# peakcrosser7/spmv-samples

Hardware: NVIDIA B200
Metric: SpMV GFLOP/s and achieved HBM GB/s vs roofline at 1/2/4/8 B200 (higher is better)
Workload: dtype f32

## Files before the change

### include/spmv_b200.h

```cpp
#ifndef SPMV_B200_H_
#define SPMV_B200_H_

#include <stddef.h>
#include <stdint.h>

#ifdef __cplusplus
extern "C" {
#endif

#define SPMVB200_API __attribute__((visibility("default")))

typedef void *spmvb200_stream_t;

enum {
    SPMVB200_OK = 0,
    SPMVB200_ERR_INVALID = 1,
    SPMVB200_ERR_ALIGNMENT = 2,
    SPMVB200_ERR_CUDA = 3,
    SPMVB200_ERR_UNSUPPORTED = 4,
    SPMVB200_ERR_CUSPARSE = 5
};

enum {
    SPMVB200_KIND_MERGE = 0,
// ... 98 lines not shown
    int64_t n_rows;
    int64_t nnz;
    int64_t max_row_len;
    int64_t empty_rows;
    double mean_row_len;
    double std_row_len;
    int32_t chosen_kind;
    int32_t chosen_width;
} spmvb200_row_stats_t;
SPMVB200_API int spmvb200_row_stats(int offset_bits, int64_t n_rows, int64_t nnz, const void *Ap,
                                    spmvb200_row_stats_t *out, spmvb200_stream_t stream);

SPMVB200_API int spmvb200_set_option(const char *name, int64_t value);
SPMVB200_API int64_t spmvb200_get_option(const char *name);
SPMVB200_API int64_t spmvb200_launch_count(void);
SPMVB200_API void spmvb200_release_cache(void);

SPMVB200_API int spmvb200_gather_yardstick(int64_t x_elements, int64_t gathers, int reps,
                                           spmvb200_stream_t stream, double *best_ms);

SPMVB200_API int spmvb200_hot_x_info(const int32_t *Aj, int64_t *hot_columns, double *hot_share,
                                     double *build_ms);
SPMVB200_API int spmvb200_hot_x_table_info(const int32_t *Aj, int64_t *table_columns, double *table_share);

typedef struct spmvb200_matrix spmvb200_matrix_t;
SPMVB200_API int spmvb200_matrix_create(int offset_bits, int value_bits, int64_t n_rows,
                                        int64_t n_cols, int64_t nnz, const void *Ap_host,
                                        const int32_t *Aj_host, const void *Ax_host,
                                        spmvb200_matrix_t **out);
SPMVB200_API int spmvb200_matrix_create_from_device(int offset_bits, int value_bits, int64_t n_rows,
                                                    int64_t n_cols, int64_t nnz, const void *Ap_dev,
                                                    const int32_t *Aj_dev, const void *Ax_dev,
                                                    spmvb200_matrix_t **out);
SPMVB200_API int spmvb200_matrix_spmv_host(spmvb200_matrix_t *m, int kind, const void *x_host,
                                           void *y_host);
#define SPMVB200_MAX_SLOTS 4
SPMVB200_API int spmvb200_matrix_submit_host(spmvb200_matrix_t *m, int kind, int slot,
                                             const void *x_host, void *y_host);
SPMVB200_API int spmvb200_matrix_wait(spmvb200_matrix_t *m, int slot);
SPMVB200_API void spmvb200_matrix_destroy(spmvb200_matrix_t *m);

SPMVB200_API int spmvb200_gen_uniform_pm1(int value_bits, uint64_t seed, uint32_t stream_id,
                                          uint64_t first, int64_t count, void *out,
                                          spmvb200_stream_t stream);
SPMVB200_API int spmvb200_gen_lap2d(int offset_bits, int value_bits, int32_t grid_n, void *Ap,
                                    int32_t *Aj, void *Ax, spmvb200_stream_t stream);
// ... 56 lines not shown
```

### spmv_samples_b200/_lib.py

```python
from __future__ import annotations

import ctypes as C
import os
import subprocess

_PKG = os.path.dirname(os.path.abspath(__file__))
LIB_PATH = os.environ.get("SPMVB200_LIB") or os.path.join(_PKG, "libspmvb200.so")
CSRC = os.path.join(_PKG, "csrc")

OK = 0
KIND_MERGE, KIND_VECTOR, KIND_LIGHT, KIND_AUTO, KIND_CUSPARSE, KIND_STREAM = 0, 1, 2, 3, 4, 5
FLAG_STATIC_PATTERN = 1
SEMIRINGS = {"plus_times": 0, "min_plus": 1, "max_plus": 2, "or_and": 3}
MAX_PEERS = 8
IPC_HANDLE_BYTES = 64


class SpmvB200Error(RuntimeError):
    def __init__(self, status: int, where: str, detail: str = ""):
        self.status = status
        super().__init__(f"{where}: status {status} ({detail})")


class Args(C.Structure):
# ... 99 lines not shown
    L.spmvb200_power_run.argtypes = [C.c_void_p, C.c_int, C.POINTER(C.c_double)]
    L.spmvb200_power_sync.argtypes = [C.c_void_p]
    L.spmvb200_power_get.argtypes = [C.c_void_p, C.c_void_p, C.POINTER(C.c_double), C.POINTER(C.c_int64)]
    L.spmvb200_power_destroy.argtypes = [C.c_void_p]
    L.spmvb200_power_exchange.argtypes = [C.c_void_p]
    L.spmvb200_power_destroy.restype = None
    L.spmvb200_norm_exchange.argtypes = [C.c_int, C.c_int64, C.c_void_p, C.c_int, C.c_int, C.c_uint64,
                                         C.c_void_p, C.POINTER(C.c_void_p), C.c_void_p, C.c_void_p,
                                         C.c_void_p, C.c_void_p, C.c_void_p]
    L.spmvb200_main_kernel_time.argtypes = [C.POINTER(C.c_double), C.POINTER(C.c_int64)]
    L.spmvb200_device_malloc.argtypes = [C.c_size_t, C.POINTER(C.c_void_p)]
    L.spmvb200_device_free.argtypes = [C.c_void_p]
    L.spmvb200_matrix_spmv_host.argtypes = [C.c_void_p, C.c_int, C.c_void_p, C.c_void_p]
    L.spmvb200_matrix_submit_host.argtypes = [C.c_void_p, C.c_int, C.c_int, C.c_void_p, C.c_void_p]
    L.spmvb200_matrix_wait.argtypes = [C.c_void_p, C.c_int]
    L.spmvb200_matrix_destroy.argtypes = [C.c_void_p]
    L.spmvb200_matrix_destroy.restype = None
    L.spmvb200_ipc_export.argtypes = [C.c_void_p, C.c_char_p]
    L.spmvb200_ipc_open.argtypes = [C.c_char_p, C.POINTER(C.c_void_p)]
    L.spmvb200_ipc_close.argtypes = [C.c_void_p]
    L.spmvb200_release_cache.restype = None
    L.spmvb200_gather_yardstick.argtypes = [C.c_int64, C.c_int64, C.c_int, C.c_void_p, C.POINTER(C.c_double)]
    L.spmvb200_hot_x_table_info.argtypes = [C.c_void_p, C.POINTER(C.c_int64), C.POINTER(C.c_double)]
    L.spmvb200_hot_x_info.argtypes = [C.c_void_p, C.POINTER(C.c_int64), C.POINTER(C.c_double),
                                      C.POINTER(C.c_double)]
    for kind in ("merge", "vector", "light", "stream", "auto", "cusparse"):
        for otag, otype in (("o32", C.c_int32), ("o64", C.c_int64)):
            for vtag in ("f32", "f64"):
                fn = getattr(L, f"spmvb200_{kind}_i32_{otag}_{vtag}")
                fn.argtypes = [C.c_int32, C.c_int32, otype, C.c_void_p, C.c_void_p, C.c_void_p,
                               C.c_void_p, C.c_void_p, C.c_void_p]
                fn.restype = C.c_int
    _lib = L
    return L


def check(status: int, where: str) -> None:
    if status != OK:
        L = lib()
        detail = L.spmvb200_status_string(status).decode()
        if status in (3, 5):
            detail += ": " + L.spmvb200_last_cuda_error().decode()
        raise SpmvB200Error(status, where, detail)


def exported_symbols():
# ... 13 lines not shown
```

### spmv_samples_b200/csrc/api.cu

```cuda
#include <cstring>
#include <new>
#include <vector>

#include "common.cuh"

namespace spmvb200 {
int64_t merge_tile_items(int offset_bits);
void stats_cache_clear();
void cusparse_plan_clear();
template <typename ValT>
int gen_uniform_pm1(uint64_t, uint32_t, uint64_t, int64_t, ValT *, cudaStream_t);
template <typename OffT, typename ValT>
int gen_lap2d(int32_t, OffT *, int32_t *, ValT *, cudaStream_t);
template <typename OffT, typename ValT>
int gen_uniform_rows(int32_t, int32_t, int32_t, uint64_t, OffT *, int32_t *, ValT *, cudaStream_t);
int gen_rmat_edges(int32_t, uint64_t, uint64_t, int64_t, int32_t *, int32_t *, cudaStream_t);
template <typename OffT, typename ValT>
int coo_to_csr(int32_t, int64_t, int32_t *, int32_t *, const ValT *, OffT *, int32_t *, ValT *,
               cudaStream_t);

namespace {

inline bool aligned16(const void *p) { return (reinterpret_cast<uintptr_t>(p) & 15u) == 0; }

// ... 263 lines not shown
                              double *best_ms) {
    return gather_yardstick(x_elements, gathers, reps, static_cast<cudaStream_t>(stream), best_ms);
}

int spmvb200_hot_x_info(const int32_t *Aj, int64_t *hot_columns, double *hot_share, double *build_ms) {
    if (hot_columns) *hot_columns = 0;
    if (hot_share) *hot_share = 0.0;
    if (build_ms) *build_ms = 0.0;
    const HotPlan *plan = hot_plan_peek(Aj);
    if (plan) {
        if (hot_columns) *hot_columns = plan->K;
        if (hot_share) *hot_share = plan->hot_share;
        if (build_ms) *build_ms = plan->build_ms;
    }
    return SPMVB200_OK;
}

int spmvb200_hot_x_table_info(const int32_t *Aj, int64_t *table_columns, double *table_share) {
    if (table_columns) *table_columns = 0;
    if (table_share) *table_share = 0.0;
    if (const HotPlan *plan = hot_plan_peek(Aj)) {
        if (table_columns) *table_columns = plan->K_table;
        if (table_share) *table_share = plan->table_share;
    }
    return SPMVB200_OK;
}

}

struct spmvb200_matrix {
    int offset_bits, value_bits;
    int64_t n_rows, n_cols, nnz;
    void *Ap = nullptr, *Ax = nullptr;
    int32_t *Aj = nullptr;
    bool owns_csr = true;
    void *x[SPMVB200_MAX_SLOTS] = {}, *y[SPMVB200_MAX_SLOTS] = {};
    cudaStream_t stream[SPMVB200_MAX_SLOTS] = {};
    int64_t calls = 0;
};

namespace spmvb200 {
template <typename ValT> int sum_squares(int64_t, const ValT *, double *, cudaStream_t);
template <typename ValT> int inv_sqrt(const double *, ValT *, cudaStream_t);
template <typename ValT>
int norm_exchange(int64_t, const ValT *, int, int, uint64_t, double *, void *const *, void *, double *, ValT *,
                  int *, cudaStream_t);
// ... 274 lines not shown
```

### spmv_samples_b200/csrc/common.cuh

```cuda
#pragma once

#include <cuda_runtime.h>

#include <cstdint>
#include <cstdio>

#include "../../include/spmv_b200.h"

namespace spmvb200 {

void record_cuda_error(cudaError_t e, const char *what, const char *file, int line);
void count_launch(int n = 1);

#define SPMV_CUDA_TRY(expr)                                                    \
    do {                                                                       \
        cudaError_t _e = (expr);                                               \
        if (_e != cudaSuccess) {                                               \
            ::spmvb200::record_cuda_error(_e, #expr, __FILE__, __LINE__);      \
            return SPMVB200_ERR_CUDA;                                          \
        }                                                                      \
    } while (0)

#define SPMV_TRY(expr)                          \
    do {                                        \
// ... 2 lines not shown
    } while (0)

#define SPMV_LAUNCH_CHECK()                     \
    do {                                        \
        ::spmvb200::count_launch();             \
        SPMV_CUDA_TRY(cudaGetLastError());      \
    } while (0)

struct DeviceInfo {
    int device = -1;
    int sm_count = 0;
    int max_threads_per_sm = 0;
    size_t l2_bytes = 0;
    size_t persisting_l2_max = 0;
    size_t access_window_max = 0;
    size_t smem_optin = 0;
};
int current_device_info(const DeviceInfo **out);

int apply_max_dynamic_smem(const void *kernel, int64_t bytes);
int apply_carveout(const void *kernel, int64_t percent);

enum ScratchSlot { SCRATCH_COORDS = 0, SCRATCH_CARRY_ROW, SCRATCH_CARRY_VAL, SCRATCH_COUNTER,
                   SCRATCH_STATS, SCRATCH_MISC, SCRATCH_SPMM_X, SCRATCH_SPMM_Y, SCRATCH_XHOT, SCRATCH_NORM, SCRATCH_NUM_SLOTS };
int scratch_get(cudaStream_t stream, ScratchSlot slot, size_t bytes, void **out);

struct PartitionTag {
    const void *coords, *Ap;
    int64_t n_rows, nnz, tile_items, n_coords;
    bool operator==(const PartitionTag &o) const {
        return coords == o.coords && Ap == o.Ap && n_rows == o.n_rows && nnz == o.nnz &&
               tile_items == o.tile_items && n_coords == o.n_coords;
    }
};
bool partition_tag_matches(cudaStream_t stream, const PartitionTag &tag);
void partition_tag_store(cudaStream_t stream, const PartitionTag &tag);
void scratch_release_all();

int64_t option_get(const char *name, int64_t fallback);

int side_fork(cudaStream_t stream, cudaStream_t *side);
int side_join(cudaStream_t stream);

class KernelTimerScope {
public:
    explicit KernelTimerScope(cudaStream_t s);
    ~KernelTimerScope();
// ... 39 lines not shown
template <typename OffT, typename ValT> int launch_auto(const SpmvProblem<OffT, ValT> &p);
template <typename OffT>
int launch_partition(int32_t n_rows, OffT nnz, const OffT *Ap, int64_t tile_items, int64_t n_coords,
                     int32_t *coords_x, cudaStream_t stream, bool reuse = false);
template <typename OffT>
int row_stats(int64_t n_rows, int64_t nnz, const OffT *Ap, spmvb200_row_stats_t *out,
              cudaStream_t stream, bool use_cache);
int pick_width_from_mean(double mean_row_len);
template <typename OffT, typename ValT>
int launch_spmm(int k, int32_t n_rows, int32_t n_cols, OffT nnz, const OffT *Ap, const int32_t *Aj,
                const ValT *Ax, const ValT *X, int64_t ldx, ValT *Y, int64_t ldy, const ValT *alpha_dev,
                cudaStream_t stream);

struct HotPlan {
    const int32_t *Aj2 = nullptr;
    const int32_t *hot_cols = nullptr;
    int64_t K = 0;
    int64_t K_table = 0;
    int32_t n_cols = 0;
    uint32_t threshold = 0;
    double hot_share = 0.0;
    double table_share = 0.0;
    double build_ms = 0.0;
};
int hot_plan_get(const int32_t *Aj, int64_t nnz, int32_t n_cols, int64_t k_max, int64_t k_table, cudaStream_t stream,
                 bool may_build, const HotPlan **out);
template <typename ValT> int hot_gather(const HotPlan &plan, const ValT *x, cudaStream_t stream, const ValT **x_hot);
void hot_plan_clear();
void hot_plan_drop(const int32_t *Aj);
const HotPlan *hot_plan_peek(const int32_t *Aj);

int gather_yardstick(int64_t n_x, int64_t count, int reps, cudaStream_t stream, double *best_ms);

struct LaunchCfg {
    cudaLaunchConfig_t cfg;
    cudaLaunchAttribute attrs[2];
};
void make_launch_cfg(LaunchCfg &lc, dim3 grid, dim3 block, size_t smem, cudaStream_t stream,
                     const void *x, size_t x_bytes);

#ifdef __CUDACC__

__device__ __forceinline__ uint32_t smem_u32(const void *p) {
    return static_cast<uint32_t>(__cvta_generic_to_shared(p));
}

__device__ __forceinline__ void mbar_init(uint64_t *bar, uint32_t count) {
    asm volatile("mbarrier.init.shared::cta.b64 [%0], %1;" ::"r"(smem_u32(bar)), "r"(count));
}
__device__ __forceinline__ void mbar_fence_init() {
// ... 150 lines not shown
```

### spmv_samples_b200/csrc/hotx.cu

```cuda
#include <cub/device/device_scan.cuh>
#include <cub/iterator/transform_input_iterator.cuh>

#include <map>
#include <mutex>

#include "common.cuh"

namespace spmvb200 {

namespace {

constexpr int kCountBuckets = 256;
__host__ __device__ __forceinline__ int count_bucket(uint32_t n) {
#ifdef __CUDA_ARCH__
    const int msb = 31 - __clz(n);
#else
    int msb = 0;
    while ((n >> msb) > 1u) ++msb;
#endif
    const uint32_t sub = msb >= 3 ? (n >> (msb - 3)) & 7u : (n << (3 - msb)) & 7u;
    return msb * 8 + (int)sub;
}
inline uint32_t bucket_lower_edge(int b) {
    const int msb = b / 8;
// ... 87 lines not shown
        }
    }
}

__global__ void __launch_bounds__(256)
hot_remap_kernel(const int32_t *__restrict__ Aj, int64_t nnz, const uint32_t *__restrict__ table,
                 int32_t *__restrict__ Aj2) {
    const int64_t stride = (int64_t)gridDim.x * blockDim.x * 4;
    for (int64_t k = ((int64_t)blockIdx.x * blockDim.x + threadIdx.x) * 4; k < nnz; k += stride) {
        if (k + 4 <= nnz) {
            const int4 c = *reinterpret_cast<const int4 *>(Aj + k);
            int4 o;
            o.x = (int32_t)__ldg(table + c.x);
            o.y = (int32_t)__ldg(table + c.y);
            o.z = (int32_t)__ldg(table + c.z);
            o.w = (int32_t)__ldg(table + c.w);
            *reinterpret_cast<int4 *>(Aj2 + k) = o;
        } else {
            for (int64_t j = k; j < nnz; ++j) Aj2[j] = (int32_t)__ldg(table + Aj[j]);
        }
    }
}

struct PlanEntry {
    HotPlan plan;
    int64_t nnz = 0;
    int32_t n_cols = 0;
    int64_t k_max = 0, k_table = 0;
    bool none = false;
};
using PlanKey = std::pair<int, const void *>;
std::mutex g_plan_mu;
std::map<PlanKey, PlanEntry> g_plans;

void entry_free(PlanEntry &e) {
    if (e.plan.Aj2) cudaFree(const_cast<int32_t *>(e.plan.Aj2));
    if (e.plan.hot_cols) cudaFree(const_cast<int32_t *>(e.plan.hot_cols));
    e = PlanEntry{};
}

int build(const int32_t *Aj, int64_t nnz, int32_t n_cols, int64_t k_max, int64_t k_table, cudaStream_t stream,
          PlanEntry &e) {
    const DeviceInfo *di = nullptr;
    SPMV_TRY(current_device_info(&di));
    const unsigned grid = (unsigned)di->sm_count * 8;
    cudaEvent_t t0 = nullptr, t1 = nullptr;
    SPMV_CUDA_TRY(cudaEventCreate(&t0));
    SPMV_CUDA_TRY(cudaEventCreate(&t1));
    SPMV_CUDA_TRY(cudaEventRecord(t0, stream));

    uint32_t *counts = nullptr, *rank_t = nullptr, *rank_w = nullptr;
    unsigned char *cls = nullptr;
    unsigned long long *hist = nullptr;
    void *scan_tmp = nullptr;
    auto cleanup = [&]() {
        if (counts) cudaFree(counts);
        if (rank_t) cudaFree(rank_t);
        if (rank_w) cudaFree(rank_w);
        if (cls) cudaFree(cls);
        if (hist) cudaFree(hist);
        if (scan_tmp) cudaFree(scan_tmp);
        if (t0) cudaEventDestroy(t0);
        if (t1) cudaEventDestroy(t1);
    };
#define HOT_TRY(expr)                                                   \
    do {                                                                \
        cudaError_t _e = (expr);                                        \
        if (_e != cudaSuccess) {                                        \
            record_cuda_error(_e, #expr, __FILE__, __LINE__);           \
            cleanup();                                                  \
            entry_free(e);                                              \
            if (_e == cudaErrorMemoryAllocation) {                      \
                 \
                (void)cudaGetLastError();                               \
                e.nnz = nnz;                                            \
                e.n_cols = n_cols;                                      \
                e.k_max = k_max;                                        \
                e.k_table = k_table;                                    \
                e.none = true;                                          \
                return SPMVB200_OK;                                     \
            }                                                           \
            return SPMVB200_ERR_CUDA;                                   \
        }                                                               \
    } while (0)
    HOT_TRY(cudaMalloc(&counts, (size_t)n_cols * 4));
    HOT_TRY(cudaMalloc(&hist, sizeof(unsigned long long) * 2 * kCountBuckets));
    HOT_TRY(cudaMemsetAsync(counts, 0, (size_t)n_cols * 4, stream));
    HOT_TRY(cudaMemsetAsync(hist, 0, sizeof(unsigned long long) * 2 * kCountBuckets, stream));
    hot_count_kernel<<<grid, 256, 0, stream>>>(Aj, nnz, counts);
    hot_hist_kernel<<<grid, 256, 0, stream>>>(counts, n_cols, hist, hist + kCountBuckets);
    count_launch(2);
    HOT_TRY(cudaGetLastError());
    unsigned long long h[2 * kCountBuckets];
    HOT_TRY(cudaMemcpyAsync(h, hist, sizeof(h), cudaMemcpyDeviceToHost, stream));
    HOT_TRY(cudaStreamSynchronize(stream));

    uint32_t threshold = 0, table_threshold = 0xffffffffu, part_lo = 0;
    int64_t K = 0, K_table = 0, part_take = 0;
    unsigned long long mass = 0;
    bool part_rest_hot = true;
    {
// ... 14 lines not shown
                break;
            }
            cols += (int64_t)h[b];
            m += h[kCountBuckets + b];
            threshold = bucket_lower_edge(b);
            K = cols;
            mass = m;
            if (table_open) {
                if (cols <= k_table) {
                    table_threshold = threshold;
                    K_table = cols;
                } else {
                    part_lo = threshold;
                    part_take = k_table - K_table;
                    table_open = false;
                }
            }
        }
    }
    e.nnz = nnz;
    e.n_cols = n_cols;
    e.k_max = k_max;
    e.k_table = k_table;
    if (K == 0 || (double)mass < (K == K_table + part_take ? 0.10 : 0.25) * (double)nnz) {
        cleanup();
        e.none = true;
        return SPMVB200_OK;
    }

    HOT_TRY(cudaMalloc(&rank_t, (size_t)n_cols * 4));
    HOT_TRY(cudaMalloc(&rank_w, (size_t)n_cols * 4));
    HOT_TRY(cudaMalloc(&cls, (size_t)n_cols));
    {
        size_t tmp_bytes = 0, tb = 0;
        cub::TransformInputIterator<uint32_t, InBand, const uint32_t *> in_part(counts, InBand{part_lo, table_threshold});
        cub::TransformInputIterator<uint32_t, IsClass, const unsigned char *> in_table(cls, IsClass{1});
        cub::TransformInputIterator<uint32_t, IsClass, const unsigned char *> in_rest(cls, IsClass{2});
        HOT_TRY(cub::DeviceScan::ExclusiveSum(nullptr, tmp_bytes, in_part, rank_w, (int)n_cols, stream));
        HOT_TRY(cub::DeviceScan::ExclusiveSum(nullptr, tb, in_table, rank_t, (int)n_cols, stream));
        if (tb > tmp_bytes) tmp_bytes = tb;
        HOT_TRY(cudaMalloc(&scan_tmp, tmp_bytes ? tmp_bytes : 16));
        if (part_take > 0) HOT_TRY(cub::DeviceScan::ExclusiveSum(scan_tmp, tmp_bytes, in_part, rank_w, (int)n_cols, stream));
        HOT_TRY(cudaMemsetAsync(hist, 0, sizeof(unsigned long long), stream));
        hot_class_kernel<<<grid, 256, 0, stream>>>(counts, n_cols, threshold, table_threshold, part_lo, (uint32_t)part_take,
                                                   part_rest_hot ? 2 : 0, rank_w, cls, hist);
        HOT_TRY(cub::DeviceScan::ExclusiveSum(scan_tmp, tmp_bytes, in_table, rank_t, (int)n_cols, stream));
        HOT_TRY(cub::DeviceScan::ExclusiveSum(scan_tmp, tmp_bytes, in_rest, rank_w, (int)n_cols, stream));
    }
    K_table += part_take;
    unsigned long long table_mass = 0;
    HOT_TRY(cudaMemcpyAsync(&table_mass, hist, sizeof(table_mass), cudaMemcpyDeviceToHost, stream));
    int32_t *hot_cols = nullptr, *Aj2 = nullptr;
    HOT_TRY(cudaMalloc(&hot_cols, (size_t)K * 4));
    e.plan.hot_cols = hot_cols;
    HOT_TRY(cudaMalloc(&Aj2, (size_t)(nnz > 0 ? nnz : 1) * 4));
    e.plan.Aj2 = Aj2;
    hot_remap_table_kernel<<<grid, 256, 0, stream>>>(cls, n_cols, (uint32_t)K_table, rank_t, rank_w, hot_cols);
    hot_remap_kernel<<<grid, 256, 0, stream>>>(Aj, nnz, rank_t, Aj2);
    count_launch(6);
    HOT_TRY(cudaGetLastError());
    HOT_TRY(cudaEventRecord(t1, stream));
    HOT_TRY(cudaStreamSynchronize(stream));
    float ms = 0.f;
    cudaEventElapsedTime(&ms, t0, t1);
    e.plan.K = K;
    e.plan.K_table = K_table;
    e.plan.n_cols = n_cols;
    e.plan.threshold = threshold;
    if (!part_rest_hot) mass = table_mass;
    e.plan.hot_share = (double)mass / (double)(nnz > 0 ? nnz : 1);
    e.plan.table_share = (double)table_mass / (double)(nnz > 0 ? nnz : 1);
    e.plan.build_ms = ms;
    cleanup();
#undef HOT_TRY
    return SPMVB200_OK;
}

}

void hot_plan_clear() {
    std::lock_guard<std::mutex> lk(g_plan_mu);
    for (auto &kv : g_plans) entry_free(kv.second);
    g_plans.clear();
}

int hot_plan_get(const int32_t *Aj, int64_t nnz, int32_t n_cols, int64_t k_max, int64_t k_table, cudaStream_t stream,
                 bool may_build, const HotPlan **out) {
    *out = nullptr;
    int dev = -1;
    SPMV_CUDA_TRY(cudaGetDevice(&dev));
    std::lock_guard<std::mutex> lk(g_plan_mu);
    const PlanKey key{dev, (const void *)Aj};
    auto it = g_plans.find(key);
    if (it != g_plans.end() && (it->second.nnz != nnz || it->second.n_cols != n_cols ||
                                (may_build && (it->second.k_max != k_max || it->second.k_table != k_table)))) {
        entry_free(it->second);
        g_plans.erase(it);
        it = g_plans.end();
    }
    if (it == g_plans.end()) {
        if (!may_build) return SPMVB200_OK;
        PlanEntry e;
        SPMV_TRY(build(Aj, nnz, n_cols, k_max, k_table, stream, e));
        it = g_plans.emplace(key, e).first;
    }
    if (!it->second.none) *out = &it->second.plan;
    return SPMVB200_OK;
}

const HotPlan *hot_plan_peek(const int32_t *Aj) {
    int dev = -1;
    if (cudaGetDevice(&dev) != cudaSuccess) return nullptr;
    std::lock_guard<std::mutex> lk(g_plan_mu);
    auto it = g_plans.find(PlanKey{dev, (const void *)Aj});
    return (it == g_plans.end() || it->second.none) ? nullptr : &it->second.plan;
}

void hot_plan_drop(const int32_t *Aj) {
    int dev = -1;
    if (cudaGetDevice(&dev) != cudaSuccess) return;
    std::lock_guard<std::mutex> lk(g_plan_mu);
    auto it = g_plans.find(PlanKey{dev, (const void *)Aj});
    if (it == g_plans.end()) return;
    entry_free(it->second);
    g_plans.erase(it);
}
// ... 4 lines not shown
```

### spmv_samples_b200/csrc/hotx_fill.cu

```cuda
#include "common.cuh"

namespace spmvb200 {

namespace {

template <typename ValT>
__global__ void __launch_bounds__(256)
hot_gather_kernel(const ValT *__restrict__ x, const int32_t *__restrict__ hot_cols, int64_t K,
                  ValT *__restrict__ x_hot) {
    for (int64_t r = (int64_t)blockIdx.x * blockDim.x + threadIdx.x; r < K; r += (int64_t)gridDim.x * blockDim.x)
        x_hot[r] = __ldg(x + __ldg(hot_cols + r));
}

}

template <typename ValT>
int hot_gather(const HotPlan &plan, const ValT *x, cudaStream_t stream, const ValT **x_hot) {
    const DeviceInfo *di = nullptr;
    SPMV_TRY(current_device_info(&di));
    void *buf = nullptr;
    SPMV_TRY(scratch_get(stream, SCRATCH_XHOT, (size_t)plan.K * sizeof(ValT), &buf));
    *x_hot = static_cast<const ValT *>(buf);
    const int64_t cap = (int64_t)di->sm_count * 16;
    const int64_t fill = option_get("hot_x_fill", 0);
    if (fill == 3) return SPMVB200_OK;
    int64_t blocks = (plan.K + 255) / 256;
    if (blocks > cap) blocks = cap;
    if (fill == 1) {
        hot_gather_kernel<ValT><<<(unsigned)blocks, 256, 0, stream>>>(x, plan.hot_cols, plan.K,
                                                                      static_cast<ValT *>(buf));
        SPMV_LAUNCH_CHECK();
        return SPMVB200_OK;
    }
    cudaStream_t side = nullptr;
    SPMV_TRY(side_fork(stream, &side));
    hot_gather_kernel<ValT><<<(unsigned)blocks, 256, 0, side>>>(x, plan.hot_cols, plan.K, static_cast<ValT *>(buf));
    SPMV_LAUNCH_CHECK();
    return side_join(stream);
}
template int hot_gather<float>(const HotPlan &, const float *, cudaStream_t, const float **);
template int hot_gather<double>(const HotPlan &, const double *, cudaStream_t, const double **);

}
```

### spmv_samples_b200/csrc/merge.cu

```cuda
#include <climits>

#include "common.cuh"

namespace spmvb200 {

namespace {

#ifndef SPMV_MERGE_BLOCK
#define SPMV_MERGE_BLOCK 256
#endif
constexpr int kMergeBlock = SPMV_MERGE_BLOCK;
constexpr int kMergeIPT = 8;
constexpr int kSlots = kMergeBlock * kMergeIPT;
constexpr int kMergeTile = kSlots - 4;
constexpr int kPad = 8;

template <typename OffT, typename ValT>
constexpr size_t merge_smem_bytes() {
    return 16 + (size_t)(kSlots + kPad) * sizeof(OffT) + (size_t)kSlots * (sizeof(int32_t) + sizeof(ValT) + 1);
}

template <typename OffT>
__global__ void __launch_bounds__(256)
merge_partition_kernel(int32_t n_rows, OffT nnz, const OffT *__restrict__ Ap, int64_t tile_items,
// ... 960 lines not shown
    } else {
        const bool has_peers = p.peers.n != 0;
        const int64_t algo_opt = option_get("merge_algo", -1);
        const bool flags_form = algo_opt < 0 ? sizeof(ValT) == 4 : algo_opt == 1;
        const bool occ = sizeof(ValT) == 4 && (sizeof(OffT) == 4 || !flags_form);
        const bool mc_f32 = p.peers.n < 0 && sizeof(ValT) == 4 && flags_form;
        const int64_t hot_opt = option_get("hot_x", -1);
        const int64_t tbl_opt = option_get("hot_x_table", -1);
        const DeviceInfo *tdi = nullptr;
        SPMV_TRY(current_device_info(&tdi));
        const bool tbl_ok = RB == kTableBlock &&
                            (tbl_opt > 0 || (tbl_opt < 0 && sizeof(ValT) == 4 && flags_form &&
                                             num_tiles >= (int64_t)tdi->sm_count * kTableGroups * 4));
        constexpr int64_t tile_smem = (int64_t)sizeof(TileSmem<kTableBlock, ValT>) * kTableGroups;
        const bool big_x = (int64_t)p.n_cols * (int64_t)sizeof(ValT) > option_get("hot_x_min_bytes", 256ll << 20);
        int64_t tbl_bytes = option_get("hot_x_table_bytes", -1);
        if (tbl_bytes < 0) tbl_bytes = big_x ? 99 << 10 : 163 << 10;
        if (tbl_bytes > 226 << 10) tbl_bytes = 226 << 10;
        tbl_bytes = (tbl_bytes + 1024) / kTableCtas - 1024;
        const int64_t k_table = tbl_ok && tbl_bytes > tile_smem ? (tbl_bytes - tile_smem) / (int64_t)sizeof(ValT) : 0;
        const bool want_hot = hot_opt > 0 || (hot_opt < 0 && p.reuse_partition && (big_x || k_table > 0));
        const int64_t k_max = (hot_opt > 0 || big_x) ? option_get("hot_x_max_bytes", 32 << 20) / (int64_t)sizeof(ValT)
                                                     : k_table;
        const HotPlan *hot = nullptr;
        if (want_hot) SPMV_TRY(hot_plan_get(p.Aj, (int64_t)p.nnz, p.n_cols, k_max, k_table, p.stream, true, &hot));
        else if (hot_opt < 0 && !p.reuse_partition) hot_plan_drop(p.Aj);
        make_launch_cfg(lc, dim3((unsigned)num_tiles), dim3(RB), 0, p.stream, p.x,
                        (size_t)p.n_cols * sizeof(ValT));
        if (hot) {
            const ValT *x_hot = nullptr;
            SPMV_TRY(hot_gather<ValT>(*hot, p.x, p.stream, &x_hot));
            const ValT *x_hot_biased = x_hot - ((ptrdiff_t)1 << 31);
            if (k_table > 0 && hot->K_table > 0) {
                auto tkernel = p.peers.n < 0 ? merge_tile_table_kernel<2, OffT, ValT>
                               : has_peers   ? merge_tile_table_kernel<1, OffT, ValT>
                                             : merge_tile_table_kernel<0, OffT, ValT>;
                int64_t tn = hot->K_table < k_table ? hot->K_table : k_table;
                const int64_t cap = option_get("hot_x_table_limit", -1);
                if (cap >= 0 && cap < tn) tn = cap;
                const uint32_t table_n = (uint32_t)tn;
                const size_t smem = (size_t)tile_smem + (size_t)table_n * sizeof(ValT);
                SPMV_TRY(apply_max_dynamic_smem(reinterpret_cast<const void *>(tkernel), (int64_t)smem));
                const DeviceInfo *di = tdi;
                const int64_t want_ctas = (num_tiles + kTableGroups - 1) / kTableGroups;
                const int64_t max_ctas = (int64_t)di->sm_count * kTableCtas;
                make_launch_cfg(lc, dim3((unsigned)(want_ctas < max_ctas ? want_ctas : max_ctas)),
                                dim3(kTableGroups * kTableBlock), smem, p.stream, p.x, (size_t)p.n_cols * sizeof(ValT));
                KernelTimerScope timed(p.stream);
                SPMV_CUDA_TRY(cudaLaunchKernelEx(&lc.cfg, tkernel, p.n_rows, p.nnz, p.Ap, hot->Aj2, p.Ax, p.x, p.y,
                                                 p.alpha_dev, p.peers, (const int32_t *)coords,
                                                 static_cast<int32_t *>(crow), static_cast<ValT *>(cval),
                                                 x_hot_biased, x_hot, table_n, num_tiles));
            } else {
            auto kernel = flags_form ? (mc_f32    ? merge_tile_hot_kernel<1, RB, 2, OffT, ValT>
                                        : has_peers ? merge_tile_hot_kernel<1, RB, 1, OffT, ValT>
                                                  : merge_tile_hot_kernel<1, RB, 0, OffT, ValT>)
                                     : (has_peers ? merge_tile_hot_kernel<0, RB, 1, OffT, ValT>
                                        : occ     ? merge_tile_hot_kernel_occ8<0, RB, 0, OffT, ValT>
                                                  : merge_tile_hot_kernel<0, RB, 0, OffT, ValT>);
            SPMV_TRY(apply_carveout(reinterpret_cast<const void *>(kernel), carveout));
            KernelTimerScope timed(p.stream);
            SPMV_CUDA_TRY(cudaLaunchKernelEx(&lc.cfg, kernel, p.n_rows, p.nnz, p.Ap, hot->Aj2, p.Ax, p.x, p.y,
                                             p.alpha_dev, p.peers, (const int32_t *)coords,
                                             static_cast<int32_t *>(crow), static_cast<ValT *>(cval),
                                             x_hot_biased));
            }
        } else {
            auto kernel = flags_form ? (mc_f32    ? merge_tile_reg_kernel<1, RB, 2, OffT, ValT>
                                        : has_peers ? merge_tile_reg_kernel<1, RB, 1, OffT, ValT>
                                        : occ     ? merge_tile_reg_kernel_occ8<1, RB, 0, OffT, ValT>
                                                  : merge_tile_reg_kernel<1, RB, 0, OffT, ValT>)
                                     : (has_peers ? merge_tile_reg_kernel<0, RB, 1, OffT, ValT>
                                        : occ     ? merge_tile_reg_kernel_occ8<0, RB, 0, OffT, ValT>
                                                  : merge_tile_reg_kernel<0, RB, 0, OffT, ValT>);
            SPMV_TRY(apply_carveout(reinterpret_cast<const void *>(kernel), carveout));
            KernelTimerScope timed(p.stream);
            SPMV_CUDA_TRY(cudaLaunchKernelEx(&lc.cfg, kernel, p.n_rows, p.nnz, p.Ap, p.Aj, p.Ax, p.x, p.y,
                                             p.alpha_dev, p.peers, (const int32_t *)coords,
                                             static_cast<int32_t *>(crow), static_cast<ValT *>(cval)));
        }
    }
    SPMV_LAUNCH_CHECK();

    if (num_tiles > 1) {
        const int64_t blocks = (num_tiles + 255) / 256;
// ... 14 lines not shown
```

### spmv_samples_b200/csrc/runtime.cu

```cuda
#include <atomic>
#include <cstdlib>
#include <cstring>
#include <map>
#include <mutex>
#include <string>
#include <utility>
#include <vector>

#include "common.cuh"

namespace spmvb200 {

namespace {
std::mutex g_mu;
thread_local char g_err[512] = "";
std::atomic<int64_t> g_launches{0};
std::map<int, DeviceInfo> g_devs;

struct ScratchBuf {
    void *ptr = nullptr;
    size_t bytes = 0;
};
struct ScratchSet {
    ScratchBuf slot[SCRATCH_NUM_SLOTS];
// ... 8 lines not shown
        {"vector_rows_per_subwarp", 0},
        {"light_width", 0},
        {"light_rows_per_claim", 0},
        {"time_main_kernel", 0},
        {"merge_carveout", -2},
        {"l2_fetch_granularity", 0},
        {"spmm_force_vector", 0},
        {"spmm_by_columns", 0},
        {"spmm_force_merge", 0},
        {"spmm_carveout", -1},
        {"merge_staging", 0},
        {"auto_kind", -1},
        {"cusparse_preprocess", 0},
        {"merge_algo", -1},
        {"hot_x", -1},
        {"hot_x_min_bytes", 256ll << 20},
        {"hot_x_table", -1},
        {"hot_x_table_limit", -1},
        {"hot_x_table_bytes", -1},
        {"assume_static_pattern", 0},
        {"side_stream", 0},
        {"hot_x_fill", 0},
        {"hot_x_max_bytes", 32ll << 20},
        {"power_exchange", -1},
        {"stream_ctas_per_sm", 3},
        {"cusparse_alg", 0},
    };
    static bool env_read = false;
    if (!env_read) {
        env_read = true;
        if (const char *e = std::getenv("SPMVB200_OPTS")) {
            std::string s(e);
            size_t pos = 0;
            while (pos < s.size()) {
                size_t end = s.find(',', pos);
                if (end == std::string::npos) end = s.size();
                const std::string kv = s.substr(pos, end - pos);
                const size_t eq = kv.find('=');
                if (eq != std::string::npos) {
                    auto it = o.find(kv.substr(0, eq));
                    if (it != o.end()) it->second = std::atoll(kv.c_str() + eq + 1);
                }
                pos = end + 1;
            }
        }
    }
// ... 290 lines not shown
```

### spmv_samples_b200/spmv.py

```python
from __future__ import annotations

import ctypes as C
import sys

import torch

from . import _lib


class SpMVKindError(ValueError):
    pass


_OFF = {torch.int32: ("o32", 32), torch.int64: ("o64", 64)}
_VAL = {torch.float32: ("f32", 32), torch.float64: ("f64", 64)}


def _ptr(t):
    return C.c_void_p(t.data_ptr() if t is not None else 0)


def _stream_ptr(stream=None):
    s = stream if stream is not None else torch.cuda.current_stream()
    return C.c_void_p(s.cuda_stream)
# ... 210 lines not shown
    _lib.check(st, "spmvb200_row_stats")
    return {f: getattr(st_out, f) for f, _ in _lib.RowStats._fields_}


def set_option(name: str, value: int) -> None:
    _lib.check(_lib.lib().spmvb200_set_option(name.encode(), int(value)), f"set_option({name})")


def get_option(name: str) -> int:
    return int(_lib.lib().spmvb200_get_option(name.encode()))


def launch_count() -> int:
    return int(_lib.lib().spmvb200_launch_count())


def hot_x_info(Aj) -> dict:
    k, share, ms = C.c_int64(0), C.c_double(0.0), C.c_double(0.0)
    with torch.cuda.device(Aj.device):
        st = _lib.lib().spmvb200_hot_x_info(_ptr(Aj), C.byref(k), C.byref(share), C.byref(ms))
        _lib.check(st, "spmvb200_hot_x_info")
        tk, tshare = C.c_int64(0), C.c_double(0.0)
        st = _lib.lib().spmvb200_hot_x_table_info(_ptr(Aj), C.byref(tk), C.byref(tshare))
    _lib.check(st, "spmvb200_hot_x_table_info")
    return {"hot_columns": int(k.value), "hot_share": float(share.value), "build_ms": float(ms.value),
            "table_columns": int(tk.value), "table_share": float(tshare.value)}


def release_cache() -> None:
    _lib.lib().spmvb200_release_cache()


def gather_yardstick(x_elements: int, gathers: int = 1 << 27, reps: int = 3, stream=None) -> float:
    ms = C.c_double(0.0)
    st = _lib.lib().spmvb200_gather_yardstick(int(x_elements), int(gathers), int(reps),
                                              _stream_ptr(stream), C.byref(ms))
    _lib.check(st, "spmvb200_gather_yardstick")
    return gathers / (ms.value * 1e-3) / 1e9
```

Before: 402.7.

## Bin cold x gathers into banded, per-call prefilled contiguous buffers for hot-x merge

Adds a plan-time pass that collects every cold (non-hot) nonzero, sorts it by nnz band and column, and rewrites Aj2 so each cold entry points at a private slot in a bins buffer. Each call, a fill kernel gathers x into those bins in column order on the side stream, and the merge kernels read x values from the bins instead of scattering into x. The aim is to turn random cold-x reads inside the main kernel into streaming reads, with the random gathers moved into a sorted, more cache-friendly prefill. The cost is an extra gather kernel plus bins traffic of about one value per cold nonzero each call, more plan build time, and extra memory. It is enabled by default only when x is large.

```diff
diff --git a/include/spmv_b200.h b/include/spmv_b200.h
--- a/include/spmv_b200.h
+++ b/include/spmv_b200.h
@@ -144,6 +144,8 @@
 SPMVB200_API int spmvb200_hot_x_info(const int32_t *Aj, int64_t *hot_columns, double *hot_share,
                                      double *build_ms);
 SPMVB200_API int spmvb200_hot_x_table_info(const int32_t *Aj, int64_t *table_columns, double *table_share);
+SPMVB200_API int spmvb200_hot_x_cold_info(const int32_t *Aj, int64_t *cold_slots, int64_t *cold_bands,
+                                          int64_t *band_nnz);
 
 typedef struct spmvb200_matrix spmvb200_matrix_t;
 SPMVB200_API int spmvb200_matrix_create(int offset_bits, int value_bits, int64_t n_rows,
diff --git a/spmv_samples_b200/_lib.py b/spmv_samples_b200/_lib.py
--- a/spmv_samples_b200/_lib.py
+++ b/spmv_samples_b200/_lib.py
@@ -145,6 +145,8 @@
     L.spmvb200_release_cache.restype = None
     L.spmvb200_gather_yardstick.argtypes = [C.c_int64, C.c_int64, C.c_int, C.c_void_p, C.POINTER(C.c_double)]
     L.spmvb200_hot_x_table_info.argtypes = [C.c_void_p, C.POINTER(C.c_int64), C.POINTER(C.c_double)]
+    L.spmvb200_hot_x_cold_info.argtypes = [C.c_void_p, C.POINTER(C.c_int64), C.POINTER(C.c_int64),
+                                           C.POINTER(C.c_int64)]
     L.spmvb200_hot_x_info.argtypes = [C.c_void_p, C.POINTER(C.c_int64), C.POINTER(C.c_double),
                                       C.POINTER(C.c_double)]
     for kind in ("merge", "vector", "light", "stream", "auto", "cusparse"):
diff --git a/spmv_samples_b200/csrc/api.cu b/spmv_samples_b200/csrc/api.cu
--- a/spmv_samples_b200/csrc/api.cu
+++ b/spmv_samples_b200/csrc/api.cu
@@ -309,6 +309,18 @@
     if (const HotPlan *plan = hot_plan_peek(Aj)) {
         if (table_columns) *table_columns = plan->K_table;
         if (table_share) *table_share = plan->table_share;
+    }
+    return SPMVB200_OK;
+}
+
+int spmvb200_hot_x_cold_info(const int32_t *Aj, int64_t *cold_slots, int64_t *cold_bands, int64_t *band_nnz) {
+    if (cold_slots) *cold_slots = 0;
+    if (cold_bands) *cold_bands = 0;
+    if (band_nnz) *band_nnz = 0;
+    if (const HotPlan *plan = hot_plan_peek(Aj)) {
+        if (cold_slots) *cold_slots = plan->n_cold;
+        if (cold_bands) *cold_bands = plan->cold_bands;
+        if (band_nnz) *band_nnz = plan->band_nnz;
     }
     return SPMVB200_OK;
 }
diff --git a/spmv_samples_b200/csrc/common.cuh b/spmv_samples_b200/csrc/common.cuh
--- a/spmv_samples_b200/csrc/common.cuh
+++ b/spmv_samples_b200/csrc/common.cuh
@@ -48,7 +48,8 @@
 int apply_carveout(const void *kernel, int64_t percent);
 
 enum ScratchSlot { SCRATCH_COORDS = 0, SCRATCH_CARRY_ROW, SCRATCH_CARRY_VAL, SCRATCH_COUNTER,
-                   SCRATCH_STATS, SCRATCH_MISC, SCRATCH_SPMM_X, SCRATCH_SPMM_Y, SCRATCH_XHOT, SCRATCH_NORM, SCRATCH_NUM_SLOTS };
+                   SCRATCH_STATS, SCRATCH_MISC, SCRATCH_SPMM_X, SCRATCH_SPMM_Y, SCRATCH_XHOT, SCRATCH_NORM, SCRATCH_BINS,
+                   SCRATCH_NUM_SLOTS };
 int scratch_get(cudaStream_t stream, ScratchSlot slot, size_t bytes, void **out);
 
 struct PartitionTag {
@@ -134,10 +135,16 @@
     double hot_share = 0.0;
     double table_share = 0.0;
     double build_ms = 0.0;
-};
-int hot_plan_get(const int32_t *Aj, int64_t nnz, int32_t n_cols, int64_t k_max, int64_t k_table, cudaStream_t stream,
-                 bool may_build, const HotPlan **out);
-template <typename ValT> int hot_gather(const HotPlan &plan, const ValT *x, cudaStream_t stream, const ValT **x_hot);
+    const int32_t *cold_cols = nullptr;
+    const int32_t *cold_slots = nullptr;
+    int64_t n_cold = 0;
+    int64_t cold_bands = 0;
+    int64_t band_nnz = 0;
+};
+int hot_plan_get(const int32_t *Aj, int64_t nnz, int32_t n_cols, int64_t k_max, int64_t k_table, int64_t bin_bytes,
+                 cudaStream_t stream, bool may_build, const HotPlan **out);
+template <typename ValT>
+int hot_gather(const HotPlan &plan, const ValT *x, cudaStream_t stream, const ValT **x_hot, const ValT **x_cold);
 void hot_plan_clear();
 void hot_plan_drop(const int32_t *Aj);
 const HotPlan *hot_plan_peek(const int32_t *Aj);
diff --git a/spmv_samples_b200/csrc/hotx.cu b/spmv_samples_b200/csrc/hotx.cu
--- a/spmv_samples_b200/csrc/hotx.cu
+++ b/spmv_samples_b200/csrc/hotx.cu
@@ -1,3 +1,6 @@
+#include <cub/block/block_reduce.cuh>
+#include <cub/block/block_scan.cuh>
+#include <cub/device/device_radix_sort.cuh>
 #include <cub/device/device_scan.cuh>
 #include <cub/iterator/transform_input_iterator.cuh>
 
@@ -133,11 +136,60 @@
     }
 }
 
+constexpr int kColdBlock = 256, kColdRounds = 16;
+constexpr int64_t kColdChunk = (int64_t)kColdBlock * kColdRounds;
+
+__global__ void __launch_bounds__(kColdBlock)
+cold_count_kernel(const int32_t *__restrict__ Aj2, int64_t nnz, unsigned long long *__restrict__ chunk_cold) {
+    using Reduce = cub::BlockReduce<uint32_t, kColdBlock>;
+    __shared__ typename Reduce::TempStorage tmp;
+    const int64_t base = (int64_t)blockIdx.x * kColdChunk;
+    uint32_t n = 0;
+    for (int j = 0; j < kColdRounds; ++j) {
+        const int64_t k = base + j * kColdBlock + threadIdx.x;
+        if (k < nnz && __ldg(Aj2 + k) >= 0) ++n;
+    }
+    n = Reduce(tmp).Sum(n);
+    if (threadIdx.x == 0) chunk_cold[blockIdx.x] = n;
+}
+
+__global__ void __launch_bounds__(kColdBlock)
+cold_keys_kernel(const int32_t *__restrict__ Aj2, int64_t nnz, const unsigned long long *__restrict__ chunk_off,
+                 int64_t band_nnz, int cbits, unsigned long long *__restrict__ keys, int64_t *__restrict__ ks) {
+    using Scan = cub::BlockScan<uint32_t, kColdBlock>;
+    __shared__ typename Scan::TempStorage tmp;
+    const int64_t base = (int64_t)blockIdx.x * kColdChunk;
+    unsigned long long off = chunk_off[blockIdx.x];
+    for (int j = 0; j < kColdRounds; ++j) {
+        const int64_t k = base + j * kColdBlock + threadIdx.x;
+        const int32_t c = k < nnz ? __ldg(Aj2 + k) : -1;
+        const uint32_t f = c >= 0 ? 1u : 0u;
+        uint32_t pos = 0, total = 0;
+        Scan(tmp).ExclusiveSum(f, pos, total);
+        if (f) {
+            keys[off + pos] = ((unsigned long long)(k / band_nnz) << cbits) | (uint32_t)c;
+            ks[off + pos] = k;
+        }
+        off += total;
+        __syncthreads();
+    }
+}
+
+__global__ void __launch_bounds__(256)
+cold_slot_kernel(const unsigned long long *__restrict__ keys, const int64_t *__restrict__ ks, int64_t n,
+                 uint32_t cmask, int32_t *__restrict__ Aj2, uint32_t *__restrict__ col, int32_t *__restrict__ slot) {
+    for (int64_t s = (int64_t)blockIdx.x * blockDim.x + threadIdx.x; s < n; s += (int64_t)gridDim.x * blockDim.x) {
+        Aj2[ks[s]] = (int32_t)s;
+        col[s] = (uint32_t)keys[s] & cmask;
+        slot[s] = (int32_t)s;
+    }
+}
+
 struct PlanEntry {
     HotPlan plan;
     int64_t nnz = 0;
     int32_t n_cols = 0;
-    int64_t k_max = 0, k_table = 0;
+    int64_t k_max = 0, k_table = 0, bin_bytes = 0;
     bool none = false;
 };
 using PlanKey = std::pair<int, const void *>;
@@ -147,11 +199,114 @@
 void entry_free(PlanEntry &e) {
     if (e.plan.Aj2) cudaFree(const_cast<int32_t *>(e.plan.Aj2));
     if (e.plan.hot_cols) cudaFree(const_cast<int32_t *>(e.plan.hot_cols));
+    if (e.plan.cold_cols) cudaFree(const_cast<int32_t *>(e.plan.cold_cols));
+    if (e.plan.cold_slots) cudaFree(const_cast<int32_t *>(e.plan.cold_slots));
     e = PlanEntry{};
 }
 
-int build(const int32_t *Aj, int64_t nnz, int32_t n_cols, int64_t k_max, int64_t k_table, cudaStream_t stream,
-          PlanEntry &e) {
+int bits_for(uint64_t v) {
+    int b = 1;
+    while (b < 64 && (v >> b) != 0) ++b;
+    return b;
+}
+
+int build_bins(int32_t *Aj2, int64_t nnz, int32_t n_cols, int64_t bin_bytes, unsigned grid, cudaStream_t stream,
+               HotPlan &plan) {
+    const int64_t n_chunks = (nnz + kColdChunk - 1) / kColdChunk;
+    if (n_chunks <= 0 || n_chunks >= 0x7fffffffLL) return SPMVB200_OK;
+    unsigned long long *chunk_cold = nullptr, *chunk_off = nullptr, *keys_a = nullptr, *keys_b = nullptr;
+    int64_t *ks_a = nullptr, *ks_b = nullptr;
+    int32_t *cols = nullptr, *slots = nullptr;
+    void *sort_tmp = nullptr, *scan_tmp = nullptr;
+    auto cleanup = [&](bool keep) {
+        for (void *q : {(void *)chunk_cold, (void *)chunk_off, (void *)keys_a, (void *)keys_b, (void *)ks_a,
+                        (void *)ks_b, sort_tmp, scan_tmp})
+            if (q) cudaFree(q);
+        if (!keep) {
+            if (cols) cudaFree(cols);
+            if (slots) cudaFree(slots);
+        }
+    };
+#define BIN_TRY(expr)                                                   \
+    do {                                                                \
+        cudaError_t _e = (expr);                                        \
+        if (_e != cudaSuccess) {                                        \
+            cleanup(false);                                             \
+            if (_e == cudaErrorMemoryAllocation) {                      \
+                (void)cudaGetLastError();                               \
+                return SPMVB200_OK;                                     \
+            }                                                           \
+            record_cuda_error(_e, #expr, __FILE__, __LINE__);           \
+            return SPMVB200_ERR_CUDA;                                   \
+        }                                                               \
+    } while (0)
+    BIN_TRY(cudaMalloc(&chunk_cold, (size_t)(n_chunks + 1) * 8));
+    BIN_TRY(cudaMalloc(&chunk_off, (size_t)(n_chunks + 1) * 8));
+    BIN_TRY(cudaMemsetAsync(chunk_cold, 0, (size_t)(n_chunks + 1) * 8, stream));
+    cold_count_kernel<<<(unsigned)n_chunks, kColdBlock, 0, stream>>>(Aj2, nnz, chunk_cold);
+    count_launch(1);
+    BIN_TRY(cudaGetLastError());
+    {
+        size_t tb = 0;
+        BIN_TRY(cub::DeviceScan::ExclusiveSum(nullptr, tb, chunk_cold, chunk_off, (int)(n_chunks + 1), stream));
+        BIN_TRY(cudaMalloc(&scan_tmp, tb ? tb : 16));
+        BIN_TRY(cub::DeviceScan::ExclusiveSum(scan_tmp, tb, chunk_cold, chunk_off, (int)(n_chunks + 1), stream));
+    }
+    unsigned long long n_cold = 0;
+    BIN_TRY(cudaMemcpyAsync(&n_cold, chunk_off + n_chunks, sizeof(n_cold), cudaMemcpyDeviceToHost, stream));
+    BIN_TRY(cudaStreamSynchronize(stream));
+    if (n_cold == 0 || n_cold > 0x7fffffffull) {
+        cleanup(false);
+        return SPMVB200_OK;
+    }
+    const int64_t n = (int64_t)n_cold;
+    const double per_band = bin_bytes >= 4 ? (double)(bin_bytes / 4) : 1.0;
+    double bn = (double)nnz * per_band / (double)n;
+    int64_t band_nnz = bn >= (double)nnz ? nnz : (int64_t)bn;
+    if (band_nnz < 1) band_nnz = 1;
+    const int64_t bands = (nnz + band_nnz - 1) / band_nnz;
+    const int cbits = bits_for((uint64_t)(n_cols > 0 ? n_cols - 1 : 0));
+    const int kbits = cbits + bits_for((uint64_t)(bands - 1));
+
+    BIN_TRY(cudaMalloc(&keys_a, (size_t)n * 8));
+    BIN_TRY(cudaMalloc(&keys_b, (size_t)n * 8));
+    BIN_TRY(cudaMalloc(&ks_a, (size_t)n * 8));
+    BIN_TRY(cudaMalloc(&ks_b, (size_t)n * 8));
+    BIN_TRY(cudaMalloc(&cols, (size_t)n * 4));
+    BIN_TRY(cudaMalloc(&slots, (size_t)n * 4));
+    uint32_t *col_in = reinterpret_cast<uint32_t *>(keys_a);
+    int32_t *slot_in = reinterpret_cast<int32_t *>(ks_a);
+    {
+        size_t t1 = 0, t2 = 0;
+        BIN_TRY(cub::DeviceRadixSort::SortPairs(nullptr, t1, keys_a, keys_b, ks_a, ks_b, (int)n, 0, kbits, stream));
+        BIN_TRY(cub::DeviceRadixSort::SortPairs(nullptr, t2, col_in, reinterpret_cast<uint32_t *>(cols), slot_in,
+                                                slots, (int)n, 0, cbits, stream));
+        if (t2 > t1) t1 = t2;
+        BIN_TRY(cudaMalloc(&sort_tmp, t1 ? t1 : 16));
+        cold_keys_kernel<<<(unsigned)n_chunks, kColdBlock, 0, stream>>>(Aj2, nnz, chunk_off, band_nnz, cbits, keys_a,
+                                                                          ks_a);
+        BIN_TRY(cudaGetLastError());
+        BIN_TRY(cub::DeviceRadixSort::SortPairs(sort_tmp, t1, keys_a, keys_b, ks_a, ks_b, (int)n, 0, kbits, stream));
+        cold_slot_kernel<<<grid, 256, 0, stream>>>(keys_b, ks_b, n, (uint32_t)((1ull << cbits) - 1), Aj2, col_in,
+                                                   slot_in);
+        BIN_TRY(cudaGetLastError());
+        BIN_TRY(cub::DeviceRadixSort::SortPairs(sort_tmp, t1, col_in, reinterpret_cast<uint32_t *>(cols), slot_in,
+                                                slots, (int)n, 0, cbits, stream));
+        count_launch(2);
+    }
+    BIN_TRY(cudaStreamSynchronize(stream));
+    cleanup(true);
+#undef BIN_TRY
+    plan.cold_cols = cols;
+    plan.cold_slots = slots;
+    plan.n_cold = n;
+    plan.cold_bands = bands;
+    plan.band_nnz = band_nnz;
+    return SPMVB200_OK;
+}
+
+int build(const int32_t *Aj, int64_t nnz, int32_t n_cols, int64_t k_max, int64_t k_table, int64_t bin_bytes,
+          cudaStream_t stream, PlanEntry &e) {
     const DeviceInfo *di = nullptr;
     SPMV_TRY(current_device_info(&di));
     const unsigned grid = (unsigned)di->sm_count * 8;
@@ -188,6 +343,7 @@
                 e.n_cols = n_cols;                                      \
                 e.k_max = k_max;                                        \
                 e.k_table = k_table;                                    \
+                e.bin_bytes = bin_bytes;                                \
                 e.none = true;                                          \
                 return SPMVB200_OK;                                     \
             }                                                           \
@@ -248,6 +404,7 @@
     e.n_cols = n_cols;
     e.k_max = k_max;
     e.k_table = k_table;
+    e.bin_bytes = bin_bytes;
     if (K == 0 || (double)mass < (K == K_table + part_take ? 0.10 : 0.25) * (double)nnz) {
         cleanup();
         e.none = true;
@@ -285,6 +442,14 @@
     hot_remap_kernel<<<grid, 256, 0, stream>>>(Aj, nnz, rank_t, Aj2);
     count_launch(6);
     HOT_TRY(cudaGetLastError());
+    if (bin_bytes > 0) {
+        const int st = build_bins(Aj2, nnz, n_cols, bin_bytes, grid, stream, e.plan);
+        if (st != SPMVB200_OK) {
+            cleanup();
+            entry_free(e);
+            return st;
+        }
+    }
     HOT_TRY(cudaEventRecord(t1, stream));
     HOT_TRY(cudaStreamSynchronize(stream));
     float ms = 0.f;
@@ -310,8 +475,8 @@
     g_plans.clear();
 }
 
-int hot_plan_get(const int32_t *Aj, int64_t nnz, int32_t n_cols, int64_t k_max, int64_t k_table, cudaStream_t stream,
-                 bool may_build, const HotPlan **out) {
+int hot_plan_get(const int32_t *Aj, int64_t nnz, int32_t n_cols, int64_t k_max, int64_t k_table, int64_t bin_bytes,
+                 cudaStream_t stream, bool may_build, const HotPlan **out) {
     *out = nullptr;
     int dev = -1;
     SPMV_CUDA_TRY(cudaGetDevice(&dev));
@@ -319,7 +484,8 @@
     const PlanKey key{dev, (const void *)Aj};
     auto it = g_plans.find(key);
     if (it != g_plans.end() && (it->second.nnz != nnz || it->second.n_cols != n_cols ||
-                                (may_build && (it->second.k_max != k_max || it->second.k_table != k_table)))) {
+                                (may_build && (it->second.k_max != k_max || it->second.k_table != k_table ||
+                                               it->second.bin_bytes != bin_bytes)))) {
         entry_free(it->second);
         g_plans.erase(it);
         it = g_plans.end();
@@ -327,7 +493,7 @@
     if (it == g_plans.end()) {
         if (!may_build) return SPMVB200_OK;
         PlanEntry e;
-        SPMV_TRY(build(Aj, nnz, n_cols, k_max, k_table, stream, e));
+        SPMV_TRY(build(Aj, nnz, n_cols, k_max, k_table, bin_bytes, stream, e));
         it = g_plans.emplace(key, e).first;
     }
     if (!it->second.none) *out = &it->second.plan;
diff --git a/spmv_samples_b200/csrc/hotx_fill.cu b/spmv_samples_b200/csrc/hotx_fill.cu
--- a/spmv_samples_b200/csrc/hotx_fill.cu
+++ b/spmv_samples_b200/csrc/hotx_fill.cu
@@ -12,33 +12,61 @@
         x_hot[r] = __ldg(x + __ldg(hot_cols + r));
 }
 
+template <typename ValT>
+__global__ void __launch_bounds__(256)
+cold_fill_kernel(const ValT *__restrict__ x, const int32_t *__restrict__ cols, const int32_t *__restrict__ slots,
+                 int64_t n, ValT *__restrict__ bins) {
+    const uint64_t pol = policy_evict_first();
+    const int64_t stride = (int64_t)gridDim.x * blockDim.x * 4;
+    for (int64_t i = ((int64_t)blockIdx.x * blockDim.x + threadIdx.x) * 4; i < n; i += stride) {
+        if (i + 4 <= n) {
+            const int4 c = ldg_stream_int4(cols + i, pol);
+            const int4 s = ldg_stream_int4(slots + i, pol);
+            const ValT v0 = __ldg(x + c.x), v1 = __ldg(x + c.y), v2 = __ldg(x + c.z), v3 = __ldg(x + c.w);
+            bins[s.x] = v0;
+            bins[s.y] = v1;
+            bins[s.z] = v2;
+            bins[s.w] = v3;
+        } else {
+            for (int64_t j = i; j < n; ++j) bins[__ldg(slots + j)] = __ldg(x + __ldg(cols + j));
+        }
+    }
+}
+
 }
 
 template <typename ValT>
-int hot_gather(const HotPlan &plan, const ValT *x, cudaStream_t stream, const ValT **x_hot) {
+int hot_gather(const HotPlan &plan, const ValT *x, cudaStream_t stream, const ValT **x_hot, const ValT **x_cold) {
     const DeviceInfo *di = nullptr;
     SPMV_TRY(current_device_info(&di));
     void *buf = nullptr;
     SPMV_TRY(scratch_get(stream, SCRATCH_XHOT, (size_t)plan.K * sizeof(ValT), &buf));
     *x_hot = static_cast<const ValT *>(buf);
+    *x_cold = x;
+    void *bins = nullptr;
+    if (plan.n_cold > 0) {
+        SPMV_TRY(scratch_get(stream, SCRATCH_BINS, (size_t)plan.n_cold * sizeof(ValT), &bins));
+        *x_cold = static_cast<const ValT *>(bins);
+    }
     const int64_t cap = (int64_t)di->sm_count * 16;
     const int64_t fill = option_get("hot_x_fill", 0);
     if (fill == 3) return SPMVB200_OK;
     int64_t blocks = (plan.K + 255) / 256;
     if (blocks > cap) blocks = cap;
-    if (fill == 1) {
-        hot_gather_kernel<ValT><<<(unsigned)blocks, 256, 0, stream>>>(x, plan.hot_cols, plan.K,
-                                                                      static_cast<ValT *>(buf));
-        SPMV_LAUNCH_CHECK();
-        return SPMVB200_OK;
-    }
-    cudaStream_t side = nullptr;
-    SPMV_TRY(side_fork(stream, &side));
+    cudaStream_t side = stream;
+    if (fill != 1) SPMV_TRY(side_fork(stream, &side));
     hot_gather_kernel<ValT><<<(unsigned)blocks, 256, 0, side>>>(x, plan.hot_cols, plan.K, static_cast<ValT *>(buf));
     SPMV_LAUNCH_CHECK();
-    return side_join(stream);
+    if (plan.n_cold > 0) {
+        int64_t cblocks = (plan.n_cold + 1023) / 1024;
+        if (cblocks > cap) cblocks = cap;
+        cold_fill_kernel<ValT><<<(unsigned)cblocks, 256, 0, side>>>(x, plan.cold_cols, plan.cold_slots, plan.n_cold,
+                                                                     static_cast<ValT *>(bins));
+        SPMV_LAUNCH_CHECK();
+    }
+    return fill == 1 ? SPMVB200_OK : side_join(stream);
 }
-template int hot_gather<float>(const HotPlan &, const float *, cudaStream_t, const float **);
-template int hot_gather<double>(const HotPlan &, const double *, cudaStream_t, const double **);
+template int hot_gather<float>(const HotPlan &, const float *, cudaStream_t, const float **, const float **);
+template int hot_gather<double>(const HotPlan &, const double *, cudaStream_t, const double **, const double **);
 
 }
diff --git a/spmv_samples_b200/csrc/merge.cu b/spmv_samples_b200/csrc/merge.cu
--- a/spmv_samples_b200/csrc/merge.cu
+++ b/spmv_samples_b200/csrc/merge.cu
@@ -1006,14 +1006,18 @@
         const bool want_hot = hot_opt > 0 || (hot_opt < 0 && p.reuse_partition && (big_x || k_table > 0));
         const int64_t k_max = (hot_opt > 0 || big_x) ? option_get("hot_x_max_bytes", 32 << 20) / (int64_t)sizeof(ValT)
                                                      : k_table;
+        const int64_t bins_opt = option_get("hot_x_cold_bins", -1);
+        const int64_t bin_bytes = bins_opt > 0 || (bins_opt < 0 && big_x) ? option_get("hot_x_bin_bytes", 8 << 20) : 0;
         const HotPlan *hot = nullptr;
-        if (want_hot) SPMV_TRY(hot_plan_get(p.Aj, (int64_t)p.nnz, p.n_cols, k_max, k_table, p.stream, true, &hot));
+        if (want_hot)
+            SPMV_TRY(hot_plan_get(p.Aj, (int64_t)p.nnz, p.n_cols, k_max, k_table, bin_bytes > 0 ? bin_bytes : 0,
+                                  p.stream, true, &hot));
         else if (hot_opt < 0 && !p.reuse_partition) hot_plan_drop(p.Aj);
         make_launch_cfg(lc, dim3((unsigned)num_tiles), dim3(RB), 0, p.stream, p.x,
                         (size_t)p.n_cols * sizeof(ValT));
         if (hot) {
-            const ValT *x_hot = nullptr;
-            SPMV_TRY(hot_gather<ValT>(*hot, p.x, p.stream, &x_hot));
+            const ValT *x_hot = nullptr, *x_cold = nullptr;
+            SPMV_TRY(hot_gather<ValT>(*hot, p.x, p.stream, &x_hot, &x_cold));
             const ValT *x_hot_biased = x_hot - ((ptrdiff_t)1 << 31);
             if (k_table > 0 && hot->K_table > 0) {
                 auto tkernel = p.peers.n < 0 ? merge_tile_table_kernel<2, OffT, ValT>
@@ -1031,7 +1035,7 @@
                 make_launch_cfg(lc, dim3((unsigned)(want_ctas < max_ctas ? want_ctas : max_ctas)),
                                 dim3(kTableGroups * kTableBlock), smem, p.stream, p.x, (size_t)p.n_cols * sizeof(ValT));
                 KernelTimerScope timed(p.stream);
-                SPMV_CUDA_TRY(cudaLaunchKernelEx(&lc.cfg, tkernel, p.n_rows, p.nnz, p.Ap, hot->Aj2, p.Ax, p.x, p.y,
+                SPMV_CUDA_TRY(cudaLaunchKernelEx(&lc.cfg, tkernel, p.n_rows, p.nnz, p.Ap, hot->Aj2, p.Ax, x_cold, p.y,
                                                  p.alpha_dev, p.peers, (const int32_t *)coords,
                                                  static_cast<int32_t *>(crow), static_cast<ValT *>(cval),
                                                  x_hot_biased, x_hot, table_n, num_tiles));
@@ -1044,7 +1048,7 @@
                                                   : merge_tile_hot_kernel<0, RB, 0, OffT, ValT>);
             SPMV_TRY(apply_carveout(reinterpret_cast<const void *>(kernel), carveout));
             KernelTimerScope timed(p.stream);
-            SPMV_CUDA_TRY(cudaLaunchKernelEx(&lc.cfg, kernel, p.n_rows, p.nnz, p.Ap, hot->Aj2, p.Ax, p.x, p.y,
+            SPMV_CUDA_TRY(cudaLaunchKernelEx(&lc.cfg, kernel, p.n_rows, p.nnz, p.Ap, hot->Aj2, p.Ax, x_cold, p.y,
                                              p.alpha_dev, p.peers, (const int32_t *)coords,
                                              static_cast<int32_t *>(crow), static_cast<ValT *>(cval),
                                              x_hot_biased));
diff --git a/spmv_samples_b200/csrc/runtime.cu b/spmv_samples_b200/csrc/runtime.cu
--- a/spmv_samples_b200/csrc/runtime.cu
+++ b/spmv_samples_b200/csrc/runtime.cu
@@ -54,6 +54,8 @@
         {"side_stream", 0},
         {"hot_x_fill", 0},
         {"hot_x_max_bytes", 32ll << 20},
+        {"hot_x_cold_bins", -1},
+        {"hot_x_bin_bytes", 8ll << 20},
         {"power_exchange", -1},
         {"stream_ctas_per_sm", 3},
         {"cusparse_alg", 0},
diff --git a/spmv_samples_b200/spmv.py b/spmv_samples_b200/spmv.py
--- a/spmv_samples_b200/spmv.py
+++ b/spmv_samples_b200/spmv.py
@@ -256,9 +256,14 @@
         _lib.check(st, "spmvb200_hot_x_info")
         tk, tshare = C.c_int64(0), C.c_double(0.0)
         st = _lib.lib().spmvb200_hot_x_table_info(_ptr(Aj), C.byref(tk), C.byref(tshare))
-    _lib.check(st, "spmvb200_hot_x_table_info")
+        _lib.check(st, "spmvb200_hot_x_table_info")
+        slots, bands, band_nnz = C.c_int64(0), C.c_int64(0), C.c_int64(0)
+        st = _lib.lib().spmvb200_hot_x_cold_info(_ptr(Aj), C.byref(slots), C.byref(bands), C.byref(band_nnz))
+    _lib.check(st, "spmvb200_hot_x_cold_info")
     return {"hot_columns": int(k.value), "hot_share": float(share.value), "build_ms": float(ms.value),
-            "table_columns": int(tk.value), "table_share": float(tshare.value)}
+            "table_columns": int(tk.value), "table_share": float(tshare.value),
+            "cold_slots": int(slots.value), "cold_bands": int(bands.value), "cold_band_nnz": int(band_nnz.value),
+            "cold_bin_bytes_f32": 4 * int(slots.value)}
 
 
 def release_cache() -> None:
```

After: 342.1 (median of 6 runs). -15.1%, worse.
